# TorontoDeepLearning/convnet

Measured on NVIDIA H100. Metric: images/sec ImageNet AlexNet training, higher is better.
Workload: dtype bf16

## Files before the change

convnet_b200/csrc/conv_kernels.h:

```cpp
#pragma once
#include <cuda_bf16.h>

#include "common.cuh"
#include "geom.h"

namespace cnb {

void simt_conv_up(const ConvGeom& g, const float* images, const float* filters, float* targets,
                  float scaleTargets, float scaleOutput, const Fuse& fuse);
void simt_conv_down(const ConvGeom& g, const float* derivs, const float* filters, float* targets,
                    float scaleTargets, float scaleOutput, const Fuse& fuse);
void simt_conv_outp(const ConvGeom& g, const float* images, const float* derivs, float* targets,
                    int rectH, int rectW, bool keep_partials, float scaleTargets, float scaleOutput);
void scale_buffer(float* a, long long n, float s);
void reduce_partials(const float* part, float* out, long long elems, int groups, int per, float st, float so);

struct ConvOutcome { int path = kPathNone; bool emitted = false, dropped = false; };
ConvOutcome tc_conv_up(const ConvGeom& g, const float* images, const float* filters, float* targets,
                       float scaleTargets, float scaleOutput, const Fuse& fuse, __nv_bfloat16* targets_bf16);
void dropout_apply(float* x, long long n, float dropprob, float scale, unsigned long long seed, __nv_bfloat16* out16);
void tc_conv_down_prestage(const ConvGeom& g, const float* derivs, const float* filters);
ConvOutcome tc_conv_down(const ConvGeom& g, const float* derivs, const float* filters, float* targets,
                         float scaleTargets, float scaleOutput, const Fuse& fuse, __nv_bfloat16* targets_bf16);
ConvPath tc_conv_outp(const ConvGeom& g, const float* images, const float* derivs, float* targets,
                      float scaleTargets, float scaleOutput);

bool want_bf16();
void to_bf16(const float* src, __nv_bfloat16* dst, long long n);
const __nv_bfloat16* bf16_staged(const float* src, long long n);
void bf16_stage(const float* ptr, long long n);
void bf16_ensure(const float* ptr, long long n);
void bf16_invalidate(const float* ptr);
void bf16_note_write(const float* ptr, long long n);
__nv_bfloat16* bf16_emit_slot(const float* ptr, long long n);
__nv_bfloat16* bf16_refresh_slot(const float* ptr, long long n);
void bf16_release();
constexpr int kMaxDgradPhases = 16;
struct DgradPhase {
  int a, b;
  int rx, ry;
  int ku, kv;
  int px, py;
  int Wp, Hp;
  long long offset;
};
struct DgradBanks { int count; DgradPhase phase[kMaxDgradPhases]; };
int dgrad_phases(const ConvGeom& g, DgradBanks* b);
const __nv_bfloat16* dgrad_weights(const float* filters, const ConvGeom& g, const DgradBanks& b, bool prestage);
uint16_t* pool_masks_slot(const float* acts, long long n_out, const float* images, long long n_in, unsigned long long sig);
const uint16_t* pool_masks_find(const float* acts, long long n_out, const float* images, unsigned long long sig);
struct Emit {
  float* target; long long n; bool want; __nv_bfloat16* buf = nullptr; bool done = false;
// ... 39 lines not shown
```

convnet_b200/csrc/conv_tc.cu:

```cuda
#include <cuda.h>
#include <cuda_bf16.h>
#include <cudaTypedefs.h>

#include <algorithm>
#include <vector>

#include "conv_kernels.h"
#include "sm90_ptx.cuh"

namespace cnb {

namespace {

constexpr int kConsumerWarps = 8;
template <int SW> constexpr int kThreadsFor = 32 * (kConsumerWarps + 1 + SW);
constexpr int BM = 128;
constexpr int BN_MAX = 128;
constexpr int BK = 32;
constexpr int kMaxStages = 8;
constexpr uint32_t kAStageBytes = BM * 128;
constexpr uint32_t kBStageBytes = BN_MAX * 128;

enum Op { kFprop = 0, kDgrad = 1, kWgrad = 2 };

struct TcParams {
  int bf16, chunk, chunk_shift, cpt, bk, nbc;
  int N, nb;
  int W, H, modX, modY, modules;
  int Cin, Cout;
  int kx, ky, sx, sy, px, py, taps;
  int frames, frame0;
  int BN, stages;
  int m_tiles, n_tiles, num_tiles;
  int kc_blocks;
  int x_mode, x_yblocks, x_ct;
  const float* xw;
  uint32_t bank_bytes;
  uint32_t epi_bytes;
  uint32_t b_tx_bytes;
  int a_merged, b_merged;
  int untied;
  int total_chunks;
  int splits, units_per_split;
  long long part_stride;
  float* out;
  __nv_bfloat16* out16;
  int vec;
  float st, so;
  const float* bias; int act;
// ... 92 lines not shown
__device__ __forceinline__ WgradSpan wgrad_span(const TcParams& p, const Tile& t) {
  WgradSpan s;
  const int tx = t.tap % p.kx, ty = t.tap / p.kx;
  s.r0 = t.split * p.units_per_split;
  s.r1 = min(s.r0 + p.units_per_split, p.modY * p.frames);
  const int lo = -(p.px + tx);
  s.mx_lo = lo <= 0 ? 0 : (lo + p.sx - 1) / p.sx;
  const int hi = p.W - 1 - p.px - tx;
  s.mx_hi = hi < 0 ? -1 : min(hi / p.sx, p.modX - 1);
  s.live_rows = 0;
  if (s.mx_hi >= s.mx_lo)
    for (int r = s.r0; r < s.r1; r++) s.live_rows += wgrad_row_live(p, r, ty) ? 1 : 0;
  return s;
}

template <int OP>
__device__ __forceinline__ int tile_kblocks(const TcParams& p, const Tile& tile) {
  if (OP == kFprop) {
    const int kcb = p.splits > 1 ? min(p.units_per_split, p.kc_blocks - tile.split * p.units_per_split) : p.kc_blocks;
    return p.x_mode ? p.Cin * p.x_yblocks : p.taps * kcb;
  } else if (OP == kDgrad) {
    const DgradTaps own = dgrad_taps(p, decode_chunks(p, tile.m_tile, p.W * p.H));
    const int kcb = p.splits > 1 ? min(p.units_per_split, p.kc_blocks - tile.split * p.units_per_split) : p.kc_blocks;
    return max(dgrad_live_taps(p, own), 1) * kcb;
  } else if (p.untied) {
    return p.nbc;
  } else if (p.x_mode) {
    const int r0 = tile.split * p.units_per_split, r1 = min(r0 + p.units_per_split, p.modY * p.frames);
    return (r1 - r0) * p.modX * p.nb;
  } else {
    const WgradSpan sp = wgrad_span(p, tile);
    return max(sp.live_rows * (sp.mx_hi - sp.mx_lo + 1), 1) * p.nbc;
  }
}

__device__ __forceinline__ uint32_t off_kmajor(int row, int k) {
  return (uint32_t)(row * 128 + ((((k >> 2) ^ row) & 7) << 4) + ((k & 3) << 2));
}
__device__ __forceinline__ uint32_t off_mnmajor(int row, int k) {
// ... 31 lines not shown
      a[ks][0] = ptx::lds32(A + off_mnmajor(row0, k0));
      a[ks][1] = ptx::lds32(A + off_mnmajor(row0 + 8, k0));
      a[ks][2] = ptx::lds32(A + off_mnmajor(row0, k0 + 1));
      a[ks][3] = ptx::lds32(A + off_mnmajor(row0 + 8, k0 + 1));
    }
    ptx::wgmma_fence();
    const uint64_t db = db0 + ((uint32_t)kb * (N * 128) >> 4);
#pragma unroll
    for (int ks = 0; ks < 4; ks++) ptx::wgmma_m64nNk8_tf32_rs<N>(acc, a[ks], db + (ks * 32 >> 4));
    ptx::wgmma_commit();
    ptx::wgmma_wait<0>();
    if (lane == 0) ptx::mbar_arrive(&ctl->empty[stage]);
    if (++stage == p.stages) { stage = 0; phase ^= 1; }
  }
  ptx::wgmma_fence_operands(acc);
}

__device__ __forceinline__ uint32_t epi_off(int row, int col) {
  return (uint32_t)(col * (BM * 4) + ((((row >> 2) ^ col) & 7) << 4) + (((row >> 2) & ~7) << 4) + ((row & 3) << 2));
}

constexpr int kWgradPassCols = 32;
constexpr uint32_t kWgradWarpBytes = 16 * kWgradPassCols * 4;
constexpr uint32_t kWgradStageBytes = kConsumerWarps * kWgradWarpBytes;
__device__ __forceinline__ uint32_t wgrad_stage_off(int row, int col) {
  return (uint32_t)(col * 64 + ((((row >> 2) ^ (col >> 1)) & 3) << 4) + ((row & 3) << 2));
}

__device__ __forceinline__ float4 ld4(const float* a, bool vec) {
  if (vec) return *reinterpret_cast<const float4*>(a);
// ... 132 lines not shown
          if (vec) {
            uint2 w;
            w.x = *reinterpret_cast<const uint32_t*>(&lo);
            w.y = *reinterpret_cast<const uint32_t*>(&hi);
            *reinterpret_cast<uint2*>(d16) = w;
          } else {
            d16[0] = lo.x; d16[1] = lo.y; d16[2] = hi.x; d16[3] = hi.y;
          }
        }
      }
    }
    phase ^= 1;
  }
}

template <int OP, bool BF16, bool SIG, int SW>
__global__ void __launch_bounds__(kThreadsFor<SW>, 1)
tc_conv_kernel(const __grid_constant__ CUtensorMap mapA, const __grid_constant__ CUtensorMap mapB, const __grid_constant__ TcParams p) {
  extern __shared__ uint8_t smem_raw[];
  uint8_t* smem = reinterpret_cast<uint8_t*>((reinterpret_cast<uintptr_t>(smem_raw) + 1023) & ~uintptr_t(1023));
  uint8_t* smemA = smem;
  uint8_t* smemB = smem + (size_t)p.stages * kAStageBytes;
  uint8_t* smemE = smemB + (p.bank_bytes ? (size_t)p.bank_bytes : (size_t)p.stages * kBStageBytes);
  SmemCtl* ctl = reinterpret_cast<SmemCtl*>(smemE + p.epi_bytes);

  const int warp = __shfl_sync(0xffffffffu, (int)(threadIdx.x >> 5), 0), lane = threadIdx.x & 31;

  if (threadIdx.x == 0) {
    for (int s = 0; s < p.stages; s++) { ptx::mbar_init(&ctl->full[s], 1); ptx::mbar_init(&ctl->empty[s], kConsumerWarps); }
    ptx::mbar_init(&ctl->epi_full, kConsumerWarps);
    ptx::mbar_init(&ctl->epi_empty, SW);
// ... 41 lines not shown
        }
        if (p.x_mode) {
          for (int c = 0; c < p.Cin; c++)
            for (int yb = 0; yb < p.x_yblocks; yb++) {
              uint8_t* a = begin_stage();
              if (p.a_merged) {
                lda5(&mapA, a, 0, cX[0], cY[0] + 4 * yb, ch.n[0] >> 5, c);
              } else {
#pragma unroll
                for (int q = 0; q < 4; q++)
                  lda5(&mapA, a + q * (BK * 128), ch.n[q], c, cX[q], cY[q] + 4 * yb, ch.f[q]);
              }
              end_stage();
            }
        } else {
          const int cb0 = p.splits > 1 ? tile.split * p.units_per_split : 0;
          const int cb1 = p.splits > 1 ? min(cb0 + p.units_per_split, p.kc_blocks) : p.kc_blocks;
          const int mod = ch.pos[0];
          for (int ty = 0; ty < p.ky; ty++)
            for (int tx = 0; tx < p.kx; tx++) {
              const int tap = tx + p.kx * ty;
              for (int cb = cb0; cb < cb1; cb++) {
                uint8_t* a = begin_stage();
                uint8_t* b = smemB + (size_t)stage * kBStageBytes;
                if (p.a_merged) {
                  lda5(&mapA, a, 0, cb * p.bk, ch.n[0] >> p.chunk_shift, cX[0] + tx, cY[0] + ty);
                } else {
#pragma unroll
                  for (int c = 0; c < 4; c++)
                    if (c < p.cpt) lda5(&mapA, a + c * (p.bk * 128), ch.n[c], cb * p.bk, cX[c] + tx, cY[c] + ty, ch.f[c]);
                }
                const int o0 = tile.n_tile * p.BN;
                if (p.b_merged) {
                  if (p.untied) lda5(&mapB, b, 0, cb * p.bk, o0 >> p.chunk_shift, tap, mod);
                  else lda4(&mapB, b, 0, cb * p.bk, o0 >> p.chunk_shift, tap);
                } else {
                  for (int j = 0; j < ((p.BN + p.chunk - 1) >> p.chunk_shift); j++) {
                    if (p.untied) lda4(&mapB, b + j * (p.bk * 128), o0 + j * p.chunk, tap, cb * p.bk, mod);
                    else lda3(&mapB, b + j * (p.bk * 128), o0 + j * p.chunk, tap, cb * p.bk);
                  }
                }
                end_stage();
              }
            }
        }
      } else if (OP == kDgrad) {
        const Chunks ch = decode_chunks(p, tile.m_tile, p.W * p.H);
        const DgradTaps taps = dgrad_taps(p, ch);
        const bool none = dgrad_live_taps(p, taps) == 0;
        int cX[4], cY[4];
#pragma unroll
        for (int c = 0; c < 4; c++) { cX[c] = ch.pos[c] % p.W; cY[c] = ch.pos[c] / p.W; }
        const int ob0 = p.splits > 1 ? tile.split * p.units_per_split : 0;
        const int ob1 = p.splits > 1 ? min(ob0 + p.units_per_split, p.kc_blocks) : p.kc_blocks;
        for (int ty = 0; ty < p.ky; ty++)
          for (int tx = 0; tx < p.kx; tx++) {
            if (!(taps.any(tx, ty) || (none && tx == 0 && ty == 0))) continue;
            int mx[4], my[4];
#pragma unroll
            for (int c = 0; c < 4; c++) {
              const bool lv = ch.ok[c] && taps.live(c, tx, ty);
              mx[c] = lv ? (cX[c] - p.px - tx) / p.sx : -1;
              my[c] = lv ? (cY[c] - p.py - ty) / p.sy : -1;
            }
            const int tap = tx + p.kx * ty;
            const int mod = mx[0] >= 0 ? mx[0] + p.modX * my[0] : -1;
            for (int ob = ob0; ob < ob1; ob++) {
              uint8_t* a = begin_stage();
              uint8_t* b = smemB + (size_t)stage * kBStageBytes;
// ... 70 lines not shown
  const int g = lane >> 2, tq = lane & 3;
  const int row0 = warp * 16 + g;
  int stage = 0; uint32_t phase = 0;
  int bank_tile = -1;
  uint32_t epi_phase = 0;
  for (int t = blockIdx.x; t < p.num_tiles; t += gridDim.x) {
    const Tile tile = decode_tile<OP>(p, t);
    const int nkb = tile_kblocks<OP>(p, tile);
    float acc[BN_MAX / 8][4];
#pragma unroll
    for (int j = 0; j < BN_MAX / 8; j++)
#pragma unroll
      for (int e = 0; e < 4; e++) acc[j][e] = 0.f;

    if constexpr (BF16 || OP == kWgrad) {
      constexpr bool a_mn = (OP != kWgrad), b_mn = (OP == kFprop);
      constexpr uint32_t a_step = a_mn ? 2048u : 32u, b_step = b_mn ? 2048u : 32u;
      const uint64_t da0 = ptx::gmma_desc(ptx::smem_u32(smemA) + (uint32_t)(warp >> 2) * 8192u, a_mn ? 8192u : 16u, 1024u);
      const uint64_t db0 = ptx::gmma_desc(ptx::smem_u32(smemB), b_mn ? 8192u : 16u, 1024u);
      int prev = -1;
      ptx::wgmma_fence_operands(acc);
      for (int kb = 0; kb < nkb; kb++) {
        ptx::mbar_wait(&ctl->full[stage], phase);
        ptx::wgmma_fence();
        const uint64_t da = da0 + ((uint32_t)stage * kAStageBytes >> 4), db = db0 + ((uint32_t)stage * kBStageBytes >> 4);
#pragma unroll
        for (int ks = 0; ks < 4; ks++) {
          if constexpr (BF16)
            ptx::wgmma_m64n128k16_bf16<a_mn ? 1 : 0, b_mn ? 1 : 0>(acc, da + (ks * a_step >> 4), db + (ks * b_step >> 4));
          else
            ptx::wgmma_m64n128k8_tf32(acc, da + (ks * a_step >> 4), db + (ks * b_step >> 4));
        }
        ptx::wgmma_commit();
        ptx::wgmma_wait<1>();
        if (prev >= 0 && lane == 0) ptx::mbar_arrive(&ctl->empty[prev]);
        prev = stage;
        if (++stage == p.stages) { stage = 0; phase ^= 1; }
      }
      ptx::wgmma_wait<0>();
      ptx::wgmma_fence_operands(acc);
      if (prev >= 0 && lane == 0) ptx::mbar_arrive(&ctl->empty[prev]);
    } else if (OP == kFprop && p.x_mode) {
      if (tile.n_tile != bank_tile) {
        ptx::bar_sync(1, 32 * kConsumerWarps);
        xmode_fill_bank(p, smemB, tile.n_tile);
        ptx::fence_proxy_async_smem();
        ptx::bar_sync(1, 32 * kConsumerWarps);
        bank_tile = tile.n_tile;
      }
      const uint32_t sA = ptx::smem_u32(smemA), bank = ptx::smem_u32(smemB);
      switch (p.BN) {
        case 32: xmode_fprop_mma<32>(acc, p, ctl, sA, bank, nkb, stage, phase, row0, tq, lane); break;
        case 64: xmode_fprop_mma<64>(acc, p, ctl, sA, bank, nkb, stage, phase, row0, tq, lane); break;
        case 96: xmode_fprop_mma<96>(acc, p, ctl, sA, bank, nkb, stage, phase, row0, tq, lane); break;
        default: xmode_fprop_mma<128>(acc, p, ctl, sA, bank, nkb, stage, phase, row0, tq, lane); break;
      }
// ... 170 lines not shown
  CUresult r = encode_fn()(map, e.bf16 ? CU_TENSOR_MAP_DATA_TYPE_BFLOAT16 : CU_TENSOR_MAP_DATA_TYPE_FLOAT32, (cuuint32_t)rank,
                           const_cast<void*>(base), gdim, gstr, bdim, estr, CU_TENSOR_MAP_INTERLEAVE_NONE,
                           CU_TENSOR_MAP_SWIZZLE_128B, CU_TENSOR_MAP_L2_PROMOTION_L2_256B, CU_TENSOR_MAP_FLOAT_OOB_FILL_NONE);
  if (r != CUDA_SUCCESS) {
    fprintf(stderr, "convnet_b200: cuTensorMapEncodeTiled failed (%d)\n", (int)r);
    return false;
  }
  return true;
}

int pick_bn(int cols, int granule) {
  const int tiles = ceil_div(cols, BN_MAX);
  const int bn = ceil_div(ceil_div(cols, tiles), granule) * granule;
  return std::min(BN_MAX, std::max(granule, bn));
}

size_t smem_bytes_for(int stages, uint32_t bank_bytes, uint32_t epi_bytes) {
  const size_t b = bank_bytes ? (size_t)bank_bytes : (size_t)stages * kBStageBytes;
  return 1024 + (size_t)stages * kAStageBytes + b + epi_bytes + sizeof(SmemCtl) + 16;
}
constexpr size_t kSmemBudget = 227 * 1024;
inline uint32_t epi_bytes_for(int bn) { return (uint32_t)BM * bn * 4; }

int pick_stages(uint32_t bank_bytes, uint32_t epi_bytes) {
  int s = kMaxStages;
  while (s > 2 && smem_bytes_for(s, bank_bytes, epi_bytes) > kSmemBudget) s--;
  return s;
}

int pick_store_warps(int kblocks, double tile_bytes) {
  const double mma_us = 0.3 * kblocks;
  const double epi_us = tile_bytes / (3e6 / 132);
  return 2.0 * epi_us >= mma_us ? 7 : 3;
}

template <int OP, bool BF16, bool SIG, int SW>
void launch_one(const CUtensorMap& a, const CUtensorMap& b, const TcParams& p, size_t smem) {
  smem_opt_in(tc_conv_kernel<OP, BF16, SIG, SW>, 227 * 1024);
  const int grid = std::min(p.num_tiles, num_sms());
  launch_pdl(tc_conv_kernel<OP, BF16, SIG, SW>, dim3((unsigned)grid), dim3(kThreadsFor<SW>), smem, state().stream, a, b, p);
}

template <int OP>
void launch(const CUtensorMap& a, const CUtensorMap& b, TcParams& p) {
  auto aligned = [](const void* q, uintptr_t a) { return (reinterpret_cast<uintptr_t>(q) & (a - 1)) == 0; };
  if (OP == kWgrad) p.epi_bytes = (!p.x_mode && p.Cout % 4 == 0 && aligned(p.out, 16)) ? kWgradStageBytes : 0u;
  else p.epi_bytes = epi_bytes_for(p.BN);
  p.stages = pick_stages(p.bank_bytes, p.epi_bytes);
  const size_t smem = smem_bytes_for(p.stages, p.bank_bytes, p.epi_bytes);
  p.vec = aligned(p.out, 16) && aligned(p.mask, 16) && aligned(p.out16, 8) ? 1 : 0;
  const bool sig = p.act == kActLogistic || (p.mask && p.mask_act == kActLogistic);
  CNB_REQUIRE(OP != kWgrad || !sig, "tc_conv: wgrad has no activation epilogue");
  void (*run)(const CUtensorMap&, const CUtensorMap&, const TcParams&, size_t) = nullptr;
  if constexpr (OP != kWgrad) {
    const int kcb = p.splits > 1 ? p.units_per_split : p.kc_blocks;
    const int kblocks = (OP == kFprop && p.x_mode) ? p.Cin * p.x_yblocks : p.taps * kcb;
    const double bytes = BM * p.BN * (4.0 + (p.out16 ? 2 : 0) + (p.mask ? 4 : 0) + (p.st != 0.f && p.splits == 1 ? 4 : 0));
    if (pick_store_warps(kblocks, bytes) == 7) {
      if (sig) run = p.bf16 ? launch_one<OP, true, true, 7> : launch_one<OP, false, true, 7>;
      else run = p.bf16 ? launch_one<OP, true, false, 7> : launch_one<OP, false, false, 7>;
    } else if (sig) {
      run = p.bf16 ? launch_one<OP, true, true, 3> : launch_one<OP, false, true, 3>;
    }
  }
  if (!run) run = p.bf16 ? launch_one<OP, true, false, 3> : launch_one<OP, false, false, 3>;
  run(a, b, p, smem);
  count_launch();
  CNB_LAUNCH_CHECK("tc_conv");
}

void fill_common(TcParams& p, const ConvGeom& g, const Elem& e) {
  p.bf16 = e.bf16; p.chunk = e.chunk; p.chunk_shift = e.shift; p.cpt = BM / e.chunk; p.bk = e.bk;
  p.N = g.N; p.nb = ceil_div(g.N, 32); p.nbc = ceil_div(g.N, e.chunk);
  p.W = g.W; p.H = g.H; p.modX = g.modX; p.modY = g.modY; p.modules = g.modules;
  p.Cin = g.Cin; p.Cout = g.Cout;
  p.kx = g.kx; p.ky = g.ky; p.sx = g.sx; p.sy = g.sy; p.px = g.px; p.py = g.py; p.taps = g.kx * g.ky;
  p.frames = g.frames; p.frame0 = 0;
  p.splits = 1; p.units_per_split = 0; p.part_stride = 0;
  p.x_mode = 0; p.x_yblocks = 0; p.x_ct = 0; p.b_tx_bytes = 0;
  p.xw = nullptr; p.bank_bytes = 0; p.epi_bytes = 0;
  p.a_merged = 0; p.b_merged = 0;
  p.untied = g.conv ? 0 : 1;
  p.bias = nullptr; p.act = 0; p.mask = nullptr; p.mask_act = 0; p.out16 = nullptr; p.vec = 0;
  p.drop_prob = 0.f; p.drop_scale = 0.f; p.drop_seed = 0;
  p.o_sx = p.o_sy = 1; p.o_x0 = p.o_y0 = 0; p.o_W = g.modX; p.out_plane = g.modules;
  p.out_frame_step = g.out_frame_step;
  p.total_chunks = 0;
  p.st = 0.f; p.so = 1.f; p.out = nullptr;
}

bool image_map(CUtensorMap* m, const void* base, const Elem& e, const ConvGeom& g, int Wd, int Hd, int C,
               long long frame_step, bool channel_second, int box_c) {
  const long long N = g.N;
  if (channel_second) {
// ... 75 lines not shown
    }
    out[i] = s;
  }
}
void reduce_split(const float* part, float* out, long long elems, int splits, float st, float so, const float* bias,
                  long long per_channel, int act, const float* mask, int mask_act) {
  const long long e4 = elems / 4;
  const int grid = (int)std::min<long long>(std::max<long long>(ceil_div<long long>(e4, 256), 1), 8LL * num_sms());
  launch_pdl(reduce_split_kernel, dim3((unsigned)grid), dim3(256), 0, state().stream, (const float4*)part, (float4*)out, e4, e4, splits,
             st, so, bias, per_channel / 4, act, (const float4*)mask, mask_act);
  count_launch();
  CNB_LAUNCH_CHECK("reduce_split");
}
void set_tiles(TcParams& p, int total_chunks, int cols, int k_channels) {
  p.kc_blocks = ceil_div(k_channels, p.bk);
  p.total_chunks = total_chunks;
  p.m_tiles = ceil_div(p.total_chunks, p.cpt);
  p.n_tiles = ceil_div(cols, p.BN);
  p.num_tiles = p.m_tiles * p.n_tiles;
  p.b_tx_bytes = p.x_mode ? 0u : (uint32_t)p.BN * 128;
}
size_t split_k(TcParams& p, const ConvGeom& g, long long out_elems, bool allowed) {
  if (!allowed || p.x_mode || p.taps != 1 || g.frames != 1 || out_elems % 4 != 0) return 0;
  if (p.num_tiles * 2 > num_sms() || p.kc_blocks < 8) return 0;
  const int ks = std::max(std::min(num_sms() / p.num_tiles, p.kc_blocks / 4), 1);
  if (ks > 1) {
    p.units_per_split = ceil_div(p.kc_blocks, ks);
    p.splits = ceil_div(p.kc_blocks, p.units_per_split);
    p.part_stride = out_elems;
    p.num_tiles *= p.splits;
// ... 99 lines not shown
  const Elem e = elem_for(true);
  const __nv_bfloat16* sd = bf16_staged(derivs, g.out_total);
  if (!sd) {
    __nv_bfloat16* tmp = (__nv_bfloat16*)workspace(align_up((size_t)g.out_total * 2));
    to_bf16(derivs, tmp, g.out_total);
    sd = tmp;
  }
  const __nv_bfloat16* bank = dgrad_weights(filters, g, banks, false);
  for (int i = 0; i < banks.count; i++) {
    const DgradPhase& P = banks.phase[i];
    TcParams p; fill_common(p, g, e);
    p.modX = P.Wp; p.modY = P.Hp; p.modules = P.Wp * P.Hp;
    p.W = g.modX; p.H = g.modY;
    p.kx = P.ku; p.ky = P.kv; p.taps = P.ku * P.kv; p.sx = p.sy = 1; p.px = P.px; p.py = P.py;
    p.Cin = g.Cout; p.Cout = g.Cin;
    p.BN = pick_bn(g.Cin, 64);
    set_tiles(p, p.nbc * p.modules, g.Cin, g.Cout);
    p.out = targets; p.st = 0.f; p.so = so;
    p.mask = fuse.act_state; p.mask_act = fuse.state_act; p.out16 = out16;
    p.o_sx = g.sx; p.o_sy = g.sy; p.o_x0 = P.a; p.o_y0 = P.b; p.o_W = g.W; p.out_plane = (long long)g.W * g.H;
    p.a_merged = 1;
    p.b_merged = (g.Cin % 64 == 0) ? 1 : 0;
    CUtensorMap fa, fb;
    if (!merged_image_map(&fa, sd, e, g, g.modX, g.modY, g.Cout, false) ||
        !filter_map(&fb, bank + P.offset, e, g.Cin, p.taps, g.Cout, p.BN, p.b_merged)) {
      CNB_REQUIRE(i == 0, "dgrad-as-fprop: tensor map failed after the first phase");
      return {};
    }
    launch<kFprop>(fa, fb, p);
  }
  return {kPathTcBf16, out16 != nullptr, false};
}

static ConvOutcome tc_conv_down_impl(const ConvGeom& g, const float* derivs, const float* filters, float* targets, float st,
                                     float so, const Fuse& fuse, __nv_bfloat16* out16, bool bf) {
  const Elem e = elem_for(bf);
  if (g.N % 4 != 0 || g.Cout % 4 != 0 || g.Cout < 8 || g.Cin < 8) return {};
  if (bf && (g.N % 8 != 0 || g.Cout % 8 != 0 || !aligned16(derivs) || !aligned16(filters))) return {};
  if (!g.conv && (g.N % 128 != 0 || g.frames != 1)) return {};
  const long long flt_n = filter_elems(g);
// ... 133 lines not shown
```

convnet_b200/csrc/sm90_ptx.cuh:

```cuda
#pragma once
#include <cuda_runtime.h>
#include <stdint.h>

namespace cnb {
namespace ptx {

__device__ __forceinline__ uint32_t smem_u32(const void* p) {
  return static_cast<uint32_t>(__cvta_generic_to_shared(p));
}

__device__ __forceinline__ void mbar_init(uint64_t* bar, uint32_t count) {
  asm volatile("mbarrier.init.shared::cta.b64 [%0], %1;" ::"r"(smem_u32(bar)), "r"(count));
}
__device__ __forceinline__ void fence_barrier_init() {
  asm volatile("fence.mbarrier_init.release.cluster;" ::: "memory");
}
__device__ __forceinline__ void mbar_arrive_expect_tx(uint64_t* bar, uint32_t bytes) {
  asm volatile("mbarrier.arrive.expect_tx.shared::cta.b64 _, [%0], %1;" ::"r"(smem_u32(bar)), "r"(bytes) : "memory");
}
__device__ __forceinline__ void mbar_arrive(uint64_t* bar) {
  asm volatile("mbarrier.arrive.shared::cta.b64 _, [%0];" ::"r"(smem_u32(bar)) : "memory");
}
__device__ __forceinline__ bool mbar_try_wait(uint64_t* bar, uint32_t parity) {
  uint32_t ok;
// ... 80 lines not shown
  return (uint64_t)((smem_addr >> 4) & 0x3FFF) | ((uint64_t)((lbo_bytes >> 4) & 0x3FFF) << 16) |
         ((uint64_t)((sbo_bytes >> 4) & 0x3FFF) << 32) | (1ULL << 62);
}
__device__ __forceinline__ void wgmma_fence() { asm volatile("wgmma.fence.sync.aligned;" ::: "memory"); }
__device__ __forceinline__ void wgmma_commit() { asm volatile("wgmma.commit_group.sync.aligned;" ::: "memory"); }
template <int N>
__device__ __forceinline__ void wgmma_wait() { asm volatile("wgmma.wait_group.sync.aligned %0;" ::"n"(N) : "memory"); }
__device__ __forceinline__ void wgmma_fence_operands(float (&d)[16][4]) {
#pragma unroll
  for (int j = 0; j < 16; j++)
#pragma unroll
    for (int e = 0; e < 4; e++) asm volatile("" : "+f"(d[j][e])::"memory");
}

#define CNB_ACC4(j) "+f"(d[j][0]), "+f"(d[j][1]), "+f"(d[j][2]), "+f"(d[j][3])
template <int TA, int TB>
__device__ __forceinline__ void wgmma_m64n128k16_bf16(float (&d)[16][4], uint64_t desc_a, uint64_t desc_b) {
  asm volatile(
      "{\n\t.reg .pred p;\n\tsetp.ne.b32 p, %68, 0;\n\t"
      "wgmma.mma_async.sync.aligned.m64n128k16.f32.bf16.bf16 "
      "{%0, %1, %2, %3, %4, %5, %6, %7, %8, %9, %10, %11, %12, %13, %14, %15, "
      "%16, %17, %18, %19, %20, %21, %22, %23, %24, %25, %26, %27, %28, %29, %30, %31, "
      "%32, %33, %34, %35, %36, %37, %38, %39, %40, %41, %42, %43, %44, %45, %46, %47, "
      "%48, %49, %50, %51, %52, %53, %54, %55, %56, %57, %58, %59, %60, %61, %62, %63}, "
      "%64, %65, p, 1, 1, %66, %67;\n\t}"
      : CNB_ACC4(0), CNB_ACC4(1), CNB_ACC4(2), CNB_ACC4(3), CNB_ACC4(4), CNB_ACC4(5), CNB_ACC4(6), CNB_ACC4(7),
        CNB_ACC4(8), CNB_ACC4(9), CNB_ACC4(10), CNB_ACC4(11), CNB_ACC4(12), CNB_ACC4(13), CNB_ACC4(14), CNB_ACC4(15)
      : "l"(desc_a), "l"(desc_b), "n"(TA), "n"(TB), "r"(1));
}

__device__ __forceinline__ void wgmma_m64n128k8_tf32(float (&d)[16][4], uint64_t desc_a, uint64_t desc_b) {
  asm volatile(
      "{\n\t.reg .pred p;\n\tsetp.ne.b32 p, %66, 0;\n\t"
      "wgmma.mma_async.sync.aligned.m64n128k8.f32.tf32.tf32 "
      "{%0, %1, %2, %3, %4, %5, %6, %7, %8, %9, %10, %11, %12, %13, %14, %15, "
      "%16, %17, %18, %19, %20, %21, %22, %23, %24, %25, %26, %27, %28, %29, %30, %31, "
      "%32, %33, %34, %35, %36, %37, %38, %39, %40, %41, %42, %43, %44, %45, %46, %47, "
      "%48, %49, %50, %51, %52, %53, %54, %55, %56, %57, %58, %59, %60, %61, %62, %63}, "
      "%64, %65, p, 1, 1;\n\t}"
      : CNB_ACC4(0), CNB_ACC4(1), CNB_ACC4(2), CNB_ACC4(3), CNB_ACC4(4), CNB_ACC4(5), CNB_ACC4(6), CNB_ACC4(7),
        CNB_ACC4(8), CNB_ACC4(9), CNB_ACC4(10), CNB_ACC4(11), CNB_ACC4(12), CNB_ACC4(13), CNB_ACC4(14), CNB_ACC4(15)
      : "l"(desc_a), "l"(desc_b), "r"(1));
}
// ... 56 lines not shown
```

convnet_b200/csrc/stage.cu:

```cuda
#include <cuda_bf16.h>

#include <vector>

#include "conv_kernels.h"

namespace cnb {

namespace {

struct Staged {
  const float* src; long long n; __nv_bfloat16* buf; size_t cap; bool valid; unsigned long long tick; int dev;
  int kind;
  unsigned long long sig;
  const float* src2; long long n2;
};
std::vector<Staged>& table() { static std::vector<Staged> t; return t; }
unsigned long long g_tick = 0;
constexpr size_t kMaxStaged = 128;

__global__ void __launch_bounds__(256) cvt_bf16_kernel(const float* __restrict__ src, __nv_bfloat16* __restrict__ dst, long long n) {
  const long long n8 = n >> 3;
  const long long stride = (long long)gridDim.x * blockDim.x;
  for (long long i = (long long)blockIdx.x * blockDim.x + threadIdx.x; i < n8; i += stride) {
    const float4 a = __ldg(reinterpret_cast<const float4*>(src) + 2 * i), b = __ldg(reinterpret_cast<const float4*>(src) + 2 * i + 1);
// ... 64 lines not shown
      if (slot->dev != dev) CNB_CUDA_CHECK(cudaSetDevice(slot->dev));
      CNB_CUDA_CHECK(cudaFree(slot->buf));
      if (slot->dev != dev) CNB_CUDA_CHECK(cudaSetDevice(dev));
    }
    slot->buf = nullptr; slot->cap = 0;
    CNB_CUDA_CHECK(cudaMalloc((void**)&slot->buf, bytes));
    slot->cap = bytes;
  }
  slot->src = ptr; slot->n = n; slot->dev = dev; slot->valid = false; slot->tick = ++g_tick; slot->kind = kind; slot->sig = sig;
  slot->src2 = nullptr; slot->n2 = 0;
  return slot;
}


__global__ void __launch_bounds__(256) dgrad_bank_kernel(const float* __restrict__ w, __nv_bfloat16* __restrict__ out, DgradBanks b,
                                                         int Cin, int Cout, int kx, int ky, int sx, int sy) {
  __shared__ float tile[32][33];
  int z = blockIdx.z, ph = 0;
  while (z >= b.phase[ph].ku * b.phase[ph].kv) { z -= b.phase[ph].ku * b.phase[ph].kv; ph++; }
  const DgradPhase& P = b.phase[ph];
  const int T = P.ku * P.kv, u = z % P.ku, v = z / P.ku;
  const int tx = P.rx + sx * (P.ku - 1 - u), ty = P.ry + sy * (P.kv - 1 - v);
  const int o0 = blockIdx.x * 32, c0 = blockIdx.y * 32;
  const int lx = threadIdx.x & 31, ly = threadIdx.x >> 5;
  for (int r = ly; r < 32; r += 8) {
    const int c = c0 + r, o = o0 + lx;
    tile[r][lx] = (c < Cin && o < Cout) ? w[o + (long long)Cout * (tx + kx * (ty + ky * c))] : 0.f;
  }
  __syncthreads();
  for (int r = ly; r < 32; r += 8) {
    const int o = o0 + r, c = c0 + lx;
    if (o < Cout && c < Cin) out[P.offset + c + (long long)Cin * (z + (long long)T * o)] = __float2bfloat16_rn(tile[lx][r]);
  }
}

}

int dgrad_phases(const ConvGeom& g, DgradBanks* b) {
  const int pad_x = -g.px, pad_y = -g.py;
  b->count = 0;
  long long off = 0;
  for (int pb = 0; pb < g.sy; pb++)
    for (int pa = 0; pa < g.sx; pa++) {
      if (pa >= g.W || pb >= g.H) continue;
      DgradPhase P;
      P.a = pa; P.b = pb;
      P.rx = (pa + pad_x) % g.sx; P.ry = (pb + pad_y) % g.sy;
// ... 7 lines not shown
      if (b->count >= kMaxDgradPhases) return -1;
      b->phase[b->count++] = P;
    }
  return b->count;
}

const __nv_bfloat16* dgrad_weights(const float* filters, const ConvGeom& g, const DgradBanks& b, bool prestage) {
  const long long n = (long long)g.Cout * g.K;
  unsigned long long sig = 1469598103934665603ULL;
  for (int v : {g.Cin, g.Cout, g.kx, g.ky, g.sx, g.sy, g.px, g.py, g.W, g.H}) sig = (sig ^ (unsigned)v) * 1099511628211ULL;
  const int dev = current_device();
  Staged* e = find_slot(filters, dev, 1, sig);
  if (e && e->valid && e->n == n) { e->tick = ++g_tick; return e->buf; }
  e = acquire_slot(filters, n, 1, sig);
  const dim3 grid((unsigned)ceil_div(g.Cout, 32), (unsigned)ceil_div(g.Cin, 32), (unsigned)(g.kx * g.ky));
  dgrad_bank_kernel<<<grid, 256, 0, state().stream>>>(filters, e->buf, b, g.Cin, g.Cout, g.kx, g.ky, g.sx, g.sy);
  count_launch();
  state().bank_builds[prestage ? 1 : 0]++;
  CNB_LAUNCH_CHECK("dgrad_banks");
  e->valid = true;
  return e->buf;
}

namespace {

}

bool want_bf16() { return state().precision == kPrecBF16; }

void to_bf16(const float* src, __nv_bfloat16* dst, long long n) {
  const long long n8 = n >> 3;
// ... 96 lines not shown
```

Baseline: 17140.

## Add N=96 wgmma, K-tail step skipping, and K-major dgrad banks

Adds bf16 wgmma variants with N=96 so tiles narrower than 128 columns stop issuing wasted MMA work. Adds a tail mode that skips k16 steps past the real channel count in the last K block. Stores dgrad weight banks K-major when Cin is not a multiple of 64, so B tiles can be 32-column granules loaded with a 3D TMA map. The cost is many more template instantiations, and the store-warp heuristic now uses scaled fractional k-block estimates.

Result: faster. 17350 (median of 6 runs) (+1.2%).

```diff
diff --git a/convnet_b200/csrc/conv_kernels.h b/convnet_b200/csrc/conv_kernels.h
--- a/convnet_b200/csrc/conv_kernels.h
+++ b/convnet_b200/csrc/conv_kernels.h
@@ -36,6 +36,7 @@
 __nv_bfloat16* bf16_refresh_slot(const float* ptr, long long n);
 void bf16_release();
 constexpr int kMaxDgradPhases = 16;
+inline bool dgrad_banks_kmajor(const ConvGeom& g) { return g.Cin % 64 != 0; }
 struct DgradPhase {
   int a, b;
   int rx, ry;
diff --git a/convnet_b200/csrc/conv_tc.cu b/convnet_b200/csrc/conv_tc.cu
--- a/convnet_b200/csrc/conv_tc.cu
+++ b/convnet_b200/csrc/conv_tc.cu
@@ -31,8 +31,11 @@
   int kx, ky, sx, sy, px, py, taps;
   int frames, frame0;
   int BN, stages;
+  int mma_n;
   int m_tiles, n_tiles, num_tiles;
   int kc_blocks;
+  int tail_ksteps;
+  int b_kmajor;
   int x_mode, x_yblocks, x_ct;
   const float* xw;
   uint32_t bank_bytes;
@@ -155,15 +158,19 @@
   return s;
 }
 
+struct KcRange { int cb0, kcb; };
+__device__ __forceinline__ KcRange tile_kc(const TcParams& p, const Tile& tile) {
+  const int cb0 = p.splits > 1 ? tile.split * p.units_per_split : 0;
+  return {cb0, p.splits > 1 ? min(p.units_per_split, p.kc_blocks - cb0) : p.kc_blocks};
+}
+
 template <int OP>
 __device__ __forceinline__ int tile_kblocks(const TcParams& p, const Tile& tile) {
   if (OP == kFprop) {
-    const int kcb = p.splits > 1 ? min(p.units_per_split, p.kc_blocks - tile.split * p.units_per_split) : p.kc_blocks;
-    return p.x_mode ? p.Cin * p.x_yblocks : p.taps * kcb;
+    return p.x_mode ? p.Cin * p.x_yblocks : p.taps * tile_kc(p, tile).kcb;
   } else if (OP == kDgrad) {
     const DgradTaps own = dgrad_taps(p, decode_chunks(p, tile.m_tile, p.W * p.H));
-    const int kcb = p.splits > 1 ? min(p.units_per_split, p.kc_blocks - tile.split * p.units_per_split) : p.kc_blocks;
-    return max(dgrad_live_taps(p, own), 1) * kcb;
+    return max(dgrad_live_taps(p, own), 1) * tile_kc(p, tile).kcb;
   } else if (p.untied) {
     return p.nbc;
   } else if (p.x_mode) {
@@ -225,6 +232,37 @@
     if (++stage == p.stages) { stage = 0; phase ^= 1; }
   }
   ptx::wgmma_fence_operands(acc);
+}
+
+template <int N, bool A_MN, bool B_MN, bool BF16, bool TAIL>
+__device__ __forceinline__ void ss_mma(float (&acc)[16][4], const TcParams& p, SmemCtl* ctl, uint64_t da0, uint64_t db0,
+                                       int nkb, int cb0, int cb1, int& stage, uint32_t& phase, int lane) {
+  constexpr uint32_t a_step = A_MN ? 2048u : 32u, b_step = B_MN ? 2048u : 32u;
+  int prev = -1, cb = cb0;
+  ptx::wgmma_fence_operands(acc);
+  for (int kb = 0; kb < nkb; kb++) {
+    const int ksteps = (TAIL && cb == p.kc_blocks - 1) ? p.tail_ksteps : 4;
+    if (++cb == cb1) cb = cb0;
+    ptx::mbar_wait(&ctl->full[stage], phase);
+    ptx::wgmma_fence();
+    const uint64_t da = da0 + ((uint32_t)stage * kAStageBytes >> 4), db = db0 + ((uint32_t)stage * kBStageBytes >> 4);
+#pragma unroll
+    for (int ks = 0; ks < 4; ks++) {
+      if (ks > 0 && ks >= ksteps) break;
+      if constexpr (BF16)
+        ptx::wgmma_m64nNk16_bf16<N, A_MN ? 1 : 0, B_MN ? 1 : 0>(acc, da + (ks * a_step >> 4), db + (ks * b_step >> 4));
+      else
+        ptx::wgmma_m64n128k8_tf32(acc, da + (ks * a_step >> 4), db + (ks * b_step >> 4));
+    }
+    ptx::wgmma_commit();
+    ptx::wgmma_wait<1>();
+    if (prev >= 0 && lane == 0) ptx::mbar_arrive(&ctl->empty[prev]);
+    prev = stage;
+    if (++stage == p.stages) { stage = 0; phase ^= 1; }
+  }
+  ptx::wgmma_wait<0>();
+  ptx::wgmma_fence_operands(acc);
+  if (prev >= 0 && lane == 0) ptx::mbar_arrive(&ctl->empty[prev]);
 }
 
 __device__ __forceinline__ uint32_t epi_off(int row, int col) {
@@ -387,7 +425,7 @@
   }
 }
 
-template <int OP, bool BF16, bool SIG, int SW>
+template <int OP, bool BF16, bool SIG, int SW, int MMA_N = 128, bool TAIL = false, bool B_KM = false>
 __global__ void __launch_bounds__(kThreadsFor<SW>, 1)
 tc_conv_kernel(const __grid_constant__ CUtensorMap mapA, const __grid_constant__ CUtensorMap mapB, const __grid_constant__ TcParams p) {
   extern __shared__ uint8_t smem_raw[];
@@ -459,8 +497,8 @@
               end_stage();
             }
         } else {
-          const int cb0 = p.splits > 1 ? tile.split * p.units_per_split : 0;
-          const int cb1 = p.splits > 1 ? min(cb0 + p.units_per_split, p.kc_blocks) : p.kc_blocks;
+          const KcRange kc = tile_kc(p, tile);
+          const int cb0 = kc.cb0, cb1 = kc.cb0 + kc.kcb;
           const int mod = ch.pos[0];
           for (int ty = 0; ty < p.ky; ty++)
             for (int tx = 0; tx < p.kx; tx++) {
@@ -476,7 +514,9 @@
                     if (c < p.cpt) lda5(&mapA, a + c * (p.bk * 128), ch.n[c], cb * p.bk, cX[c] + tx, cY[c] + ty, ch.f[c]);
                 }
                 const int o0 = tile.n_tile * p.BN;
-                if (p.b_merged) {
+                if (B_KM) {
+                  lda3(&mapB, b, cb * p.bk, tap, o0);
+                } else if (p.b_merged) {
                   if (p.untied) lda5(&mapB, b, 0, cb * p.bk, o0 >> p.chunk_shift, tap, mod);
                   else lda4(&mapB, b, 0, cb * p.bk, o0 >> p.chunk_shift, tap);
                 } else {
@@ -496,8 +536,8 @@
         int cX[4], cY[4];
 #pragma unroll
         for (int c = 0; c < 4; c++) { cX[c] = ch.pos[c] % p.W; cY[c] = ch.pos[c] / p.W; }
-        const int ob0 = p.splits > 1 ? tile.split * p.units_per_split : 0;
-        const int ob1 = p.splits > 1 ? min(ob0 + p.units_per_split, p.kc_blocks) : p.kc_blocks;
+        const KcRange kc = tile_kc(p, tile);
+        const int ob0 = kc.cb0, ob1 = kc.cb0 + kc.kcb;
         for (int ty = 0; ty < p.ky; ty++)
           for (int tx = 0; tx < p.kx; tx++) {
             if (!(taps.any(tx, ty) || (none && tx == 0 && ty == 0))) continue;
@@ -598,32 +638,12 @@
       for (int e = 0; e < 4; e++) acc[j][e] = 0.f;
 
     if constexpr (BF16 || OP == kWgrad) {
-      constexpr bool a_mn = (OP != kWgrad), b_mn = (OP == kFprop);
-      constexpr uint32_t a_step = a_mn ? 2048u : 32u, b_step = b_mn ? 2048u : 32u;
+      constexpr bool a_mn = (OP != kWgrad), b_mn = (OP == kFprop) && !B_KM;
       const uint64_t da0 = ptx::gmma_desc(ptx::smem_u32(smemA) + (uint32_t)(warp >> 2) * 8192u, a_mn ? 8192u : 16u, 1024u);
       const uint64_t db0 = ptx::gmma_desc(ptx::smem_u32(smemB), b_mn ? 8192u : 16u, 1024u);
-      int prev = -1;
-      ptx::wgmma_fence_operands(acc);
-      for (int kb = 0; kb < nkb; kb++) {
-        ptx::mbar_wait(&ctl->full[stage], phase);
-        ptx::wgmma_fence();
-        const uint64_t da = da0 + ((uint32_t)stage * kAStageBytes >> 4), db = db0 + ((uint32_t)stage * kBStageBytes >> 4);
-#pragma unroll
-        for (int ks = 0; ks < 4; ks++) {
-          if constexpr (BF16)
-            ptx::wgmma_m64n128k16_bf16<a_mn ? 1 : 0, b_mn ? 1 : 0>(acc, da + (ks * a_step >> 4), db + (ks * b_step >> 4));
-          else
-            ptx::wgmma_m64n128k8_tf32(acc, da + (ks * a_step >> 4), db + (ks * b_step >> 4));
-        }
-        ptx::wgmma_commit();
-        ptx::wgmma_wait<1>();
-        if (prev >= 0 && lane == 0) ptx::mbar_arrive(&ctl->empty[prev]);
-        prev = stage;
-        if (++stage == p.stages) { stage = 0; phase ^= 1; }
-      }
-      ptx::wgmma_wait<0>();
-      ptx::wgmma_fence_operands(acc);
-      if (prev >= 0 && lane == 0) ptx::mbar_arrive(&ctl->empty[prev]);
+      int cb0 = 0, cb1 = 1;
+      if constexpr (TAIL) { const KcRange kc = tile_kc(p, tile); cb0 = kc.cb0; cb1 = kc.cb0 + kc.kcb; }
+      ss_mma<BF16 ? MMA_N : 128, a_mn, b_mn, BF16, BF16 && TAIL>(acc, p, ctl, da0, db0, nkb, cb0, cb1, stage, phase, lane);
     } else if (OP == kFprop && p.x_mode) {
       if (tile.n_tile != bank_tile) {
         ptx::bar_sync(1, 32 * kConsumerWarps);
@@ -824,6 +844,7 @@
   const int bn = ceil_div(ceil_div(cols, tiles), granule) * granule;
   return std::min(BN_MAX, std::max(granule, bn));
 }
+int pick_mma_n(int bn, bool b_mn) { return (bn <= 96 && !b_mn) ? 96 : 128; }
 
 size_t smem_bytes_for(int stages, uint32_t bank_bytes, uint32_t epi_bytes) {
   const size_t b = bank_bytes ? (size_t)bank_bytes : (size_t)stages * kBStageBytes;
@@ -838,17 +859,32 @@
   return s;
 }
 
-int pick_store_warps(int kblocks, double tile_bytes) {
+int pick_store_warps(double kblocks, double tile_bytes) {
   const double mma_us = 0.3 * kblocks;
   const double epi_us = tile_bytes / (3e6 / 132);
   return 2.0 * epi_us >= mma_us ? 7 : 3;
 }
 
-template <int OP, bool BF16, bool SIG, int SW>
+template <int OP, bool BF16, bool SIG, int SW, int MMA_N = 128, bool TAIL = false, bool B_KM = false>
 void launch_one(const CUtensorMap& a, const CUtensorMap& b, const TcParams& p, size_t smem) {
-  smem_opt_in(tc_conv_kernel<OP, BF16, SIG, SW>, 227 * 1024);
+  constexpr auto kernel = tc_conv_kernel<OP, BF16, SIG, SW, MMA_N, TAIL, B_KM>;
+  smem_opt_in(kernel, 227 * 1024);
   const int grid = std::min(p.num_tiles, num_sms());
-  launch_pdl(tc_conv_kernel<OP, BF16, SIG, SW>, dim3((unsigned)grid), dim3(kThreadsFor<SW>), smem, state().stream, a, b, p);
+  launch_pdl(kernel, dim3((unsigned)grid), dim3(kThreadsFor<SW>), smem, state().stream, a, b, p);
+}
+using RunFn = void (*)(const CUtensorMap&, const CUtensorMap&, const TcParams&, size_t);
+template <int OP, int SW>
+RunFn bf16_instance(int n, bool tail, bool b_km) {
+  if constexpr (OP == kWgrad) {
+    return n == 96 ? launch_one<OP, true, false, SW, 96> : launch_one<OP, true, false, SW, 128>;
+  } else if constexpr (OP == kFprop) {
+    if (!b_km) return tail ? launch_one<OP, true, false, SW, 128, true> : launch_one<OP, true, false, SW, 128>;
+    if (n == 96) return tail ? launch_one<OP, true, false, SW, 96, true, true> : launch_one<OP, true, false, SW, 96, false, true>;
+    return tail ? launch_one<OP, true, false, SW, 128, true, true> : launch_one<OP, true, false, SW, 128, false, true>;
+  } else {
+    if (n == 96) return tail ? launch_one<OP, true, false, SW, 96, true> : launch_one<OP, true, false, SW, 96>;
+    return tail ? launch_one<OP, true, false, SW, 128, true> : launch_one<OP, true, false, SW, 128>;
+  }
 }
 
 template <int OP>
@@ -861,19 +897,27 @@
   p.vec = aligned(p.out, 16) && aligned(p.mask, 16) && aligned(p.out16, 8) ? 1 : 0;
   const bool sig = p.act == kActLogistic || (p.mask && p.mask_act == kActLogistic);
   CNB_REQUIRE(OP != kWgrad || !sig, "tc_conv: wgrad has no activation epilogue");
-  void (*run)(const CUtensorMap&, const CUtensorMap&, const TcParams&, size_t) = nullptr;
+  const bool b_km = OP == kFprop && p.b_kmajor;
+  p.mma_n = (p.bf16 && !sig) ? pick_mma_n(p.BN, OP == kFprop && !b_km) : BN_MAX;
+  if (!p.bf16 || sig || OP == kWgrad) p.tail_ksteps = 4;
+  const bool tail = p.tail_ksteps < 4;
+  RunFn run = nullptr;
   if constexpr (OP != kWgrad) {
     const int kcb = p.splits > 1 ? p.units_per_split : p.kc_blocks;
-    const int kblocks = (OP == kFprop && p.x_mode) ? p.Cin * p.x_yblocks : p.taps * kcb;
+    const double short_kb = p.splits > 1 ? 0.0 : (4 - p.tail_ksteps) / 4.0;
+    const double kblocks = (OP == kFprop && p.x_mode) ? p.Cin * p.x_yblocks
+                                                      : p.taps * (kcb - short_kb) * (p.bf16 ? p.mma_n / 128.0 : 1.0);
     const double bytes = BM * p.BN * (4.0 + (p.out16 ? 2 : 0) + (p.mask ? 4 : 0) + (p.st != 0.f && p.splits == 1 ? 4 : 0));
     if (pick_store_warps(kblocks, bytes) == 7) {
-      if (sig) run = p.bf16 ? launch_one<OP, true, true, 7> : launch_one<OP, false, true, 7>;
-      else run = p.bf16 ? launch_one<OP, true, false, 7> : launch_one<OP, false, false, 7>;
+      if (sig) run = !p.bf16 ? launch_one<OP, false, true, 7>
+                             : (b_km ? launch_one<OP, true, true, 7, 128, false, true> : launch_one<OP, true, true, 7>);
+      else run = p.bf16 ? bf16_instance<OP, 7>(p.mma_n, tail, b_km) : launch_one<OP, false, false, 7>;
     } else if (sig) {
-      run = p.bf16 ? launch_one<OP, true, true, 3> : launch_one<OP, false, true, 3>;
-    }
-  }
-  if (!run) run = p.bf16 ? launch_one<OP, true, false, 3> : launch_one<OP, false, false, 3>;
+      run = !p.bf16 ? launch_one<OP, false, true, 3>
+                    : (b_km ? launch_one<OP, true, true, 3, 128, false, true> : launch_one<OP, true, true, 3>);
+    }
+  }
+  if (!run) run = p.bf16 ? bf16_instance<OP, 3>(p.mma_n, tail, b_km) : launch_one<OP, false, false, 3>;
   run(a, b, p, smem);
   count_launch();
   CNB_LAUNCH_CHECK("tc_conv");
@@ -888,6 +932,7 @@
   p.frames = g.frames; p.frame0 = 0;
   p.splits = 1; p.units_per_split = 0; p.part_stride = 0;
   p.x_mode = 0; p.x_yblocks = 0; p.x_ct = 0; p.b_tx_bytes = 0;
+  p.mma_n = BN_MAX; p.tail_ksteps = 4; p.b_kmajor = 0;
   p.xw = nullptr; p.bank_bytes = 0; p.epi_bytes = 0;
   p.a_merged = 0; p.b_merged = 0;
   p.untied = g.conv ? 0 : 1;
@@ -993,6 +1038,7 @@
 }
 void set_tiles(TcParams& p, int total_chunks, int cols, int k_channels) {
   p.kc_blocks = ceil_div(k_channels, p.bk);
+  p.tail_ksteps = (p.bf16 && k_channels % p.bk != 0) ? ceil_div(k_channels % p.bk, 16) : 4;
   p.total_chunks = total_chunks;
   p.m_tiles = ceil_div(p.total_chunks, p.cpt);
   p.n_tiles = ceil_div(cols, p.BN);
@@ -1122,7 +1168,8 @@
     p.W = g.modX; p.H = g.modY;
     p.kx = P.ku; p.ky = P.kv; p.taps = P.ku * P.kv; p.sx = p.sy = 1; p.px = P.px; p.py = P.py;
     p.Cin = g.Cout; p.Cout = g.Cin;
-    p.BN = pick_bn(g.Cin, 64);
+    p.b_kmajor = dgrad_banks_kmajor(g) ? 1 : 0;
+    p.BN = pick_bn(g.Cin, p.b_kmajor ? 32 : 64);
     set_tiles(p, p.nbc * p.modules, g.Cin, g.Cout);
     p.out = targets; p.st = 0.f; p.so = so;
     p.mask = fuse.act_state; p.mask_act = fuse.state_act; p.out16 = out16;
@@ -1130,8 +1177,12 @@
     p.a_merged = 1;
     p.b_merged = (g.Cin % 64 == 0) ? 1 : 0;
     CUtensorMap fa, fb;
+    const long long bdims[3] = {g.Cout, p.taps, g.Cin};
+    const long long bstr[2] = {g.Cout, (long long)g.Cout * p.taps};
+    const int bbox[3] = {e.chunk, 1, p.BN};
     if (!merged_image_map(&fa, sd, e, g, g.modX, g.modY, g.Cout, false) ||
-        !filter_map(&fb, bank + P.offset, e, g.Cin, p.taps, g.Cout, p.BN, p.b_merged)) {
+        !(p.b_kmajor ? make_map(&fb, bank + P.offset, e, 3, bdims, bstr, bbox)
+                     : filter_map(&fb, bank + P.offset, e, g.Cin, p.taps, g.Cout, p.BN, p.b_merged))) {
       CNB_REQUIRE(i == 0, "dgrad-as-fprop: tensor map failed after the first phase");
       return {};
     }
diff --git a/convnet_b200/csrc/sm90_ptx.cuh b/convnet_b200/csrc/sm90_ptx.cuh
--- a/convnet_b200/csrc/sm90_ptx.cuh
+++ b/convnet_b200/csrc/sm90_ptx.cuh
@@ -118,19 +118,34 @@
 }
 
 #define CNB_ACC4(j) "+f"(d[j][0]), "+f"(d[j][1]), "+f"(d[j][2]), "+f"(d[j][3])
-template <int TA, int TB>
-__device__ __forceinline__ void wgmma_m64n128k16_bf16(float (&d)[16][4], uint64_t desc_a, uint64_t desc_b) {
-  asm volatile(
-      "{\n\t.reg .pred p;\n\tsetp.ne.b32 p, %68, 0;\n\t"
-      "wgmma.mma_async.sync.aligned.m64n128k16.f32.bf16.bf16 "
-      "{%0, %1, %2, %3, %4, %5, %6, %7, %8, %9, %10, %11, %12, %13, %14, %15, "
-      "%16, %17, %18, %19, %20, %21, %22, %23, %24, %25, %26, %27, %28, %29, %30, %31, "
-      "%32, %33, %34, %35, %36, %37, %38, %39, %40, %41, %42, %43, %44, %45, %46, %47, "
-      "%48, %49, %50, %51, %52, %53, %54, %55, %56, %57, %58, %59, %60, %61, %62, %63}, "
-      "%64, %65, p, 1, 1, %66, %67;\n\t}"
-      : CNB_ACC4(0), CNB_ACC4(1), CNB_ACC4(2), CNB_ACC4(3), CNB_ACC4(4), CNB_ACC4(5), CNB_ACC4(6), CNB_ACC4(7),
-        CNB_ACC4(8), CNB_ACC4(9), CNB_ACC4(10), CNB_ACC4(11), CNB_ACC4(12), CNB_ACC4(13), CNB_ACC4(14), CNB_ACC4(15)
-      : "l"(desc_a), "l"(desc_b), "n"(TA), "n"(TB), "r"(1));
+template <int N, int TA, int TB>
+__device__ __forceinline__ void wgmma_m64nNk16_bf16(float (&d)[16][4], uint64_t desc_a, uint64_t desc_b) {
+  static_assert(N == 96 || N == 128, "bf16 SS wgmma: N in {96, 128}");
+  static_assert(N % 64 == 0 || TB == 0, "MN-major B spans whole 64-column swizzle atoms");
+  if constexpr (N == 96) {
+    asm volatile(
+        "{\n\t.reg .pred p;\n\tsetp.ne.b32 p, %52, 0;\n\t"
+        "wgmma.mma_async.sync.aligned.m64n96k16.f32.bf16.bf16 "
+        "{%0, %1, %2, %3, %4, %5, %6, %7, %8, %9, %10, %11, %12, %13, %14, %15, "
+        "%16, %17, %18, %19, %20, %21, %22, %23, %24, %25, %26, %27, %28, %29, %30, %31, "
+        "%32, %33, %34, %35, %36, %37, %38, %39, %40, %41, %42, %43, %44, %45, %46, %47}, "
+        "%48, %49, p, 1, 1, %50, %51;\n\t}"
+        : CNB_ACC4(0), CNB_ACC4(1), CNB_ACC4(2), CNB_ACC4(3), CNB_ACC4(4), CNB_ACC4(5), CNB_ACC4(6), CNB_ACC4(7),
+          CNB_ACC4(8), CNB_ACC4(9), CNB_ACC4(10), CNB_ACC4(11)
+        : "l"(desc_a), "l"(desc_b), "n"(TA), "n"(TB), "r"(1));
+  } else {
+    asm volatile(
+        "{\n\t.reg .pred p;\n\tsetp.ne.b32 p, %68, 0;\n\t"
+        "wgmma.mma_async.sync.aligned.m64n128k16.f32.bf16.bf16 "
+        "{%0, %1, %2, %3, %4, %5, %6, %7, %8, %9, %10, %11, %12, %13, %14, %15, "
+        "%16, %17, %18, %19, %20, %21, %22, %23, %24, %25, %26, %27, %28, %29, %30, %31, "
+        "%32, %33, %34, %35, %36, %37, %38, %39, %40, %41, %42, %43, %44, %45, %46, %47, "
+        "%48, %49, %50, %51, %52, %53, %54, %55, %56, %57, %58, %59, %60, %61, %62, %63}, "
+        "%64, %65, p, 1, 1, %66, %67;\n\t}"
+        : CNB_ACC4(0), CNB_ACC4(1), CNB_ACC4(2), CNB_ACC4(3), CNB_ACC4(4), CNB_ACC4(5), CNB_ACC4(6), CNB_ACC4(7),
+          CNB_ACC4(8), CNB_ACC4(9), CNB_ACC4(10), CNB_ACC4(11), CNB_ACC4(12), CNB_ACC4(13), CNB_ACC4(14), CNB_ACC4(15)
+        : "l"(desc_a), "l"(desc_b), "n"(TA), "n"(TB), "r"(1));
+  }
 }
 
 __device__ __forceinline__ void wgmma_m64n128k8_tf32(float (&d)[16][4], uint64_t desc_a, uint64_t desc_b) {
diff --git a/convnet_b200/csrc/stage.cu b/convnet_b200/csrc/stage.cu
--- a/convnet_b200/csrc/stage.cu
+++ b/convnet_b200/csrc/stage.cu
@@ -102,7 +102,7 @@
 
 
 __global__ void __launch_bounds__(256) dgrad_bank_kernel(const float* __restrict__ w, __nv_bfloat16* __restrict__ out, DgradBanks b,
-                                                         int Cin, int Cout, int kx, int ky, int sx, int sy) {
+                                                         int Cin, int Cout, int kx, int ky, int sx, int sy, bool kmajor) {
   __shared__ float tile[32][33];
   int z = blockIdx.z, ph = 0;
   while (z >= b.phase[ph].ku * b.phase[ph].kv) { z -= b.phase[ph].ku * b.phase[ph].kv; ph++; }
@@ -117,8 +117,13 @@
   }
   __syncthreads();
   for (int r = ly; r < 32; r += 8) {
-    const int o = o0 + r, c = c0 + lx;
-    if (o < Cout && c < Cin) out[P.offset + c + (long long)Cin * (z + (long long)T * o)] = __float2bfloat16_rn(tile[lx][r]);
+    if (kmajor) {
+      const int c = c0 + r, o = o0 + lx;
+      if (o < Cout && c < Cin) out[P.offset + o + (long long)Cout * (z + (long long)T * c)] = __float2bfloat16_rn(tile[r][lx]);
+    } else {
+      const int o = o0 + r, c = c0 + lx;
+      if (o < Cout && c < Cin) out[P.offset + c + (long long)Cin * (z + (long long)T * o)] = __float2bfloat16_rn(tile[lx][r]);
+    }
   }
 }
 
@@ -156,7 +161,8 @@
   if (e && e->valid && e->n == n) { e->tick = ++g_tick; return e->buf; }
   e = acquire_slot(filters, n, 1, sig);
   const dim3 grid((unsigned)ceil_div(g.Cout, 32), (unsigned)ceil_div(g.Cin, 32), (unsigned)(g.kx * g.ky));
-  dgrad_bank_kernel<<<grid, 256, 0, state().stream>>>(filters, e->buf, b, g.Cin, g.Cout, g.kx, g.ky, g.sx, g.sy);
+  dgrad_bank_kernel<<<grid, 256, 0, state().stream>>>(filters, e->buf, b, g.Cin, g.Cout, g.kx, g.ky, g.sx, g.sy,
+                                                       dgrad_banks_kmajor(g));
   count_launch();
   state().bank_builds[prestage ? 1 : 0]++;
   CNB_LAUNCH_CHECK("dgrad_banks");
```
